# GinZhu/RDST

Hardware: AMD Instinct MI355X
Metric: SR patches/sec fwd+bwd, RDST-E1 x4 64->256 (higher is better)
Workload: dtype bf16; 1 GPU; RDST-E1 x4 (RDST_E1_OASIS_example_SRx4.ini), 1x64x64 LR patches -> 256x256, step = fwd + L1 + bwd + flat-bucket grad all-reduce + Adam; global_batch=32, per_gpu_batch=32, parallelism=dp1, hip_graph=True, grad_bucket_bytes=17859844

## Files before the change

### rdst_amd/csrc/reduce_batch.hip

```cpp
#include "reduce_batch.h"
#include <vector>

namespace rbatch {
namespace {

constexpr int MAXJ = 16;
struct SumBatch { SumJob j[MAXJ]; int first[MAXJ + 1]; int n; };
struct FinBatch { FinJob j[MAXJ]; int first[MAXJ + 1]; int n; };

thread_local bool g_active = false;
thread_local std::vector<SumJob> g_sums;
thread_local std::vector<FinJob> g_fins;

__device__ __forceinline__ void emit(const SumJob& J, int n, int c, int i, float a) {
  if (J.map == MAP_COPY) {
    J.out[J.g4 ? n * J.b2 + c : i] = a;
  } else if (J.map == MAP_LINEAR) {
    const int K = J.a, Kx = J.b;
    if (!J.g4) { n = i / Kx; c = i - n * Kx; }
    if (c < K) { if (J.out) J.out[(int64_t)n * K + c] = a * J.s; }
    else if (c == K && J.out2) J.out2[n] = a * J.s;
  } else if (J.map == MAP_MLP) {
    const int C = J.a, hid = J.b, n1 = hid * (C + 1);
    if (i < n1) J.out[i] = a;
    else {
      const int i2 = i - n1, jj = i2 / C, cc = i2 - jj * C;
      if (jj < hid) J.out2[(int64_t)cc * hid + jj] = a;
      else J.out3[cc] = a;
    }
  } else if (J.map == MAP_T) {
    const int rows = J.a;
    if (n < rows) J.out[(int64_t)c * rows + n] = a;
    else if (n == rows) J.out2[c] = a;
  } else {
    const int heads = J.a, T = J.b, hh = i / T, t = i - hh * T;
    J.out[t * heads + hh] = a;
  }
}

__global__ void __launch_bounds__(256) batched_sum_kernel(const SumBatch bt) {
  __shared__ float part[4][8][33];
  int k = 0;
#pragma unroll
  for (int q = 1; q < MAXJ; ++q) k += (q < bt.n && (int)blockIdx.x >= bt.first[q]) ? 1 : 0;
  const SumJob& J = bt.j[k];
  const int o = threadIdx.x & 31, sg = threadIdx.x >> 5;
  const int i = ((int)blockIdx.x - bt.first[k]) * 32 + o;
  float a0 = 0.f, a1 = 0.f, a2 = 0.f, a3 = 0.f;
  if (i < J.tot) {
    if (J.g4) {
      const uint2* sl = reinterpret_cast<const uint2*>(J.slab);
      for (int w0 = sg; w0 < J.nwg; w0 += 8 * 8) {
        uint2 v[8];
#pragma unroll
        for (int u = 0; u < 8; ++u) v[u] = (w0 + 8 * u < J.nwg) ? sl[(int64_t)(w0 + 8 * u) * J.stride + i] : make_uint2(0u, 0u);
#pragma unroll
        for (int u = 0; u < 8; ++u) {
          a0 += __uint_as_float(v[u].x << 16); a1 += __uint_as_float(v[u].x & 0xffff0000u);
          a2 += __uint_as_float(v[u].y << 16); a3 += __uint_as_float(v[u].y & 0xffff0000u);
        }
      }
    } else {
      for (int w0 = sg; w0 < J.nwg; w0 += 8 * 8) {
        float v[8];
#pragma unroll
        for (int u = 0; u < 8; ++u) v[u] = (w0 + 8 * u < J.nwg) ? J.slab[(int64_t)(w0 + 8 * u) * J.stride + i] : 0.f;
#pragma unroll
        for (int u = 0; u < 8; ++u) a0 += v[u];
      }
    }
  }
  part[0][sg][o] = a0; part[1][sg][o] = a1; part[2][sg][o] = a2; part[3][sg][o] = a3;
  __syncthreads();
  if (sg != 0 || i >= J.tot) return;
  float r[4] = {0.f, 0.f, 0.f, 0.f};
#pragma unroll
  for (int e = 0; e < 4; ++e)
#pragma unroll
    for (int q = 0; q < 8; ++q) r[e] += part[e][q][o];
  if (J.g4) {
    const int W = J.b2, ng = i / W, c = i - ng * W;
#pragma unroll
    for (int e = 0; e < 4; ++e)
      if (4 * ng + e < J.a2) emit(J, 4 * ng + e, c, 0, r[e]);
  } else {
    emit(J, 0, 0, i, r[0]);
  }
}

__global__ void __launch_bounds__(1024) batched_ln_finish_kernel(const FinBatch bt) {
  __shared__ float pg[128][9], pb[128][9], qg[8][9], qb[8][9];
  int kj = 0;
#pragma unroll
  for (int q = 1; q < MAXJ; ++q) kj += (q < bt.n && (int)blockIdx.x >= bt.first[q]) ? 1 : 0;
  const FinJob& J = bt.j[kj];
  const int tx = threadIdx.x & 7, ty = threadIdx.x >> 3;
  const int blk = (int)blockIdx.x - bt.first[kj];
  const int k = blk * 8 + tx;
  const int N = J.N, K = J.K, Kx = J.Kx;
  const float s = J.s;
  const float gk = k < K ? J.gamma[k] : 0.f, bk = k < K ? J.beta[k] : 0.f;
  float ag = 0.f, ab = 0.f;
#pragma unroll 3
  for (int n = ty; n < N; n += 128) {
    const float db = J.G[(int64_t)n * Kx + K];
    if (k < K) {
      const float g = J.G[(int64_t)n * Kx + k], w = J.Wt[(int64_t)n * K + k];
      if (J.dW) J.dW[(int64_t)n * K + k] = s * fmaf(gk, g, bk * db);
      ag = fmaf(w, g, ag);
      ab = fmaf(w, db, ab);
    }
    if (blk == 0 && tx == 0 && J.dbias) J.dbias[n] = s * db;
  }
  pg[ty][tx] = ag;
  pb[ty][tx] = ab;
  __syncthreads();
  if (ty < 8) {
    float a = 0.f, b = 0.f;
#pragma unroll
    for (int j = 0; j < 16; ++j) { a += pg[ty * 16 + j][tx]; b += pb[ty * 16 + j][tx]; }
    qg[ty][tx] = a;
    qb[ty][tx] = b;
  }
  __syncthreads();
  if (ty == 0 && k < K) {
    float a = 0.f, b = 0.f;
#pragma unroll
    for (int j = 0; j < 8; ++j) { a += qg[j][tx]; b += qb[j][tx]; }
    if (J.dgamma) J.dgamma[k] = s * a;
    if (J.dbeta) J.dbeta[k] = s * b;
  }
}

int launch_sums(const SumJob* jobs, int n, hipStream_t st) {
  for (int base = 0; base < n; base += MAXJ) {
    SumBatch bt{};
    bt.n = n - base < MAXJ ? n - base : MAXJ;
    int blocks = 0;
    for (int q = 0; q < bt.n; ++q) {
      bt.j[q] = jobs[base + q];
      bt.first[q] = blocks;
      blocks += (bt.j[q].tot + 31) / 32;
    }
    bt.first[bt.n] = blocks;
    if (blocks == 0) continue;
    hipLaunchKernelGGL(batched_sum_kernel, dim3((unsigned)blocks), dim3(256), 0, st, bt);
    if (int rc = rdst_launch_status("batched_sum")) return rc;
  }
  return 0;
}
int launch_fins(const FinJob* jobs, int n, hipStream_t st) {
  for (int base = 0; base < n; base += MAXJ) {
    FinBatch bt{};
    bt.n = n - base < MAXJ ? n - base : MAXJ;
    int blocks = 0;
    for (int q = 0; q < bt.n; ++q) {
      bt.j[q] = jobs[base + q];
      bt.first[q] = blocks;
      blocks += (bt.j[q].K + 7) / 8;
    }
    bt.first[bt.n] = blocks;
    if (blocks == 0) continue;
    hipLaunchKernelGGL(batched_ln_finish_kernel, dim3((unsigned)blocks), dim3(1024), 0, st, bt);
    if (int rc = rdst_launch_status("batched_ln_finish")) return rc;
  }
  return 0;
}

}

int sum(const SumJob& j, hipStream_t st) {
  if (g_active) { g_sums.push_back(j); return 0; }
  return launch_sums(&j, 1, st);
}
int finish(const FinJob& j, hipStream_t st) {
  if (g_active) { g_fins.push_back(j); return 0; }
  return launch_fins(&j, 1, st);
}

}

extern "C" int rdst_reduce_batch_begin(void) {
  if (rbatch::g_active) return rdst_fail(RDST_EINVAL, "rdst_reduce_batch_begin: a batch is already open on this thread");
  rbatch::g_active = true;
  rbatch::g_sums.clear();
  rbatch::g_fins.clear();
  return 0;
}

extern "C" int rdst_reduce_batch_end(void* stream) {
  if (!rbatch::g_active) return rdst_fail(RDST_EINVAL, "rdst_reduce_batch_end: no open batch");
  rbatch::g_active = false;
  hipStream_t st = (hipStream_t)stream;
  int rc = rbatch::launch_sums(rbatch::g_sums.data(), (int)rbatch::g_sums.size(), st);
  if (!rc) rc = rbatch::launch_fins(rbatch::g_fins.data(), (int)rbatch::g_fins.size(), st);
  rbatch::g_sums.clear();
  rbatch::g_fins.clear();
  return rc;
}

extern "C" int rdst_reduce_batch_abort(void) {
  rbatch::g_active = false;
  rbatch::g_sums.clear();
  rbatch::g_fins.clear();
  return 0;
}
```

Measured before the change: 1889 patches/s.

## Fuse LayerNorm backward finish into batched sum kernel via last-block tickets

Pairs each batched column-sum job with the LayerNorm finish job that consumes its output, and runs both in one kernel launch. Sum blocks are re-tiled per row and column tile; each block bumps a per-chunk atomic ticket in global memory, and the last contributor runs the gamma/beta/dW reduction for that chunk. This removes a separate finish launch and the gap between the two kernels. The cost is atomic traffic, write-through stores with acquire fences, more shared memory per block, and a ticket-slot ring that must stay consistent when the step is replayed from a HIP graph.

```diff
diff --git a/rdst_amd/csrc/reduce_batch.hip b/rdst_amd/csrc/reduce_batch.hip
--- a/rdst_amd/csrc/reduce_batch.hip
+++ b/rdst_amd/csrc/reduce_batch.hip
@@ -1,20 +1,27 @@
 #include "reduce_batch.h"
+#include <atomic>
 #include <vector>
 
 namespace rbatch {
 namespace {
 
 constexpr int MAXJ = 16;
-struct SumBatch { SumJob j[MAXJ]; int first[MAXJ + 1]; int n; };
+constexpr int TICKET_SLOTS = 64;
+struct SumBatch { SumJob j[MAXJ]; FinJob f[MAXJ]; int first[MAXJ + 1]; int n; unsigned paired; int slot; };
 struct FinBatch { FinJob j[MAXJ]; int first[MAXJ + 1]; int n; };
 
 thread_local bool g_active = false;
 thread_local std::vector<SumJob> g_sums;
 thread_local std::vector<FinJob> g_fins;
-
-__device__ __forceinline__ void emit(const SumJob& J, int n, int c, int i, float a) {
+std::atomic<unsigned> g_slot{0};
+constexpr int MAXCH = 32;
+__device__ unsigned g_tickets[TICKET_SLOTS][MAXJ][MAXCH];
+
+__device__ __forceinline__ void emit(const SumJob& J, int n, int c, int i, float a, bool wt) {
   if (J.map == MAP_COPY) {
-    J.out[J.g4 ? n * J.b2 + c : i] = a;
+    float* dst = &J.out[J.g4 ? n * J.b2 + c : i];
+    if (wt) __hip_atomic_store(reinterpret_cast<unsigned*>(dst), __float_as_uint(a), __ATOMIC_RELAXED, __HIP_MEMORY_SCOPE_AGENT);
+    else *dst = a;
   } else if (J.map == MAP_LINEAR) {
     const int K = J.a, Kx = J.b;
     if (!J.g4) { n = i / Kx; c = i - n * Kx; }
@@ -38,16 +45,85 @@
   }
 }
 
-__global__ void __launch_bounds__(256) batched_sum_kernel(const SumBatch bt) {
-  __shared__ float part[4][8][33];
+__device__ __forceinline__ void ln_finish_chunk(const FinJob& J, unsigned q, float* sh) {
+  float* pg = sh; float* pb = sh + 128 * 9; float* qg = sh + 2 * 128 * 9; float* qb = qg + 8 * 9;
+  const unsigned N = J.N, K = J.K, Kx = J.Kx;
+  const float s = J.s;
+  const float* __restrict__ G = J.G;
+  const float* __restrict__ Wt = J.Wt;
+  float* __restrict__ dW = J.dW;
+  float* __restrict__ dbias = J.dbias;
+  const unsigned tx = threadIdx.x & 7, ty0 = threadIdx.x >> 3, k = q * 8 + tx;
+  const unsigned kk = k < K ? k : K - 1;
+  const float gk = J.gamma[kk], bk = J.beta[kk];
+  float ag[4], ab[4];
+#pragma unroll
+  for (int u = 0; u < 4; ++u) ag[u] = ab[u] = 0.f;
+#pragma unroll 1
+  for (unsigned n0 = ty0; n0 < N; n0 += 128) {
+    float gg[4], w[4], db[4];
+#pragma unroll
+    for (int u = 0; u < 4; ++u) {
+      const unsigned n = n0 + 32 * u < N ? n0 + 32 * u : n0;
+      gg[u] = G[n * Kx + kk]; w[u] = Wt[n * K + kk]; db[u] = G[n * Kx + K];
+    }
+#pragma unroll
+    for (int u = 0; u < 4; ++u) {
+      const unsigned n = n0 + 32 * u;
+      if (n < N) {
+        if (k < K) {
+          if (dW) dW[n * K + k] = s * fmaf(gk, gg[u], bk * db[u]);
+          ag[u] = fmaf(w[u], gg[u], ag[u]);
+          ab[u] = fmaf(w[u], db[u], ab[u]);
+        }
+        if (q == 0 && tx == 0 && dbias) dbias[n] = s * db[u];
+      }
+    }
+  }
+#pragma unroll
+  for (int u = 0; u < 4; ++u) { pg[(ty0 + 32 * u) * 9 + tx] = ag[u]; pb[(ty0 + 32 * u) * 9 + tx] = ab[u]; }
+  __syncthreads();
+  if (ty0 < 8) {
+    float a = 0.f, b = 0.f;
+#pragma unroll
+    for (int j = 0; j < 16; ++j) { a += pg[(ty0 * 16 + j) * 9 + tx]; b += pb[(ty0 * 16 + j) * 9 + tx]; }
+    qg[ty0 * 9 + tx] = a;
+    qb[ty0 * 9 + tx] = b;
+  }
+  __syncthreads();
+  if (ty0 == 0 && k < K) {
+    float a = 0.f, b = 0.f;
+#pragma unroll
+    for (int j = 0; j < 8; ++j) { a += qg[j * 9 + tx]; b += qb[j * 9 + tx]; }
+    if (J.dgamma) J.dgamma[k] = s * a;
+    if (J.dbeta) J.dbeta[k] = s * b;
+  }
+  __syncthreads();
+}
+
+constexpr int SH_FIN = 2 * 128 * 9 + 2 * 8 * 9;
+
+__global__ void __launch_bounds__(256, 8) batched_sum_kernel(const SumBatch bt) {
+  __shared__ float sh[SH_FIN + 1];
+  float (*part)[8][33] = reinterpret_cast<float (*)[8][33]>(sh);
   int k = 0;
 #pragma unroll
   for (int q = 1; q < MAXJ; ++q) k += (q < bt.n && (int)blockIdx.x >= bt.first[q]) ? 1 : 0;
   const SumJob& J = bt.j[k];
+  const bool paired = (bt.paired >> k) & 1u;
   const int o = threadIdx.x & 31, sg = threadIdx.x >> 5;
-  const int i = ((int)blockIdx.x - bt.first[k]) * 32 + o;
+  const int blk = (int)blockIdx.x - bt.first[k];
+  int i = blk * 32 + o, tile = 0, units = 0;
+  bool live = i < J.tot;
+  if (paired) {
+    const int W = bt.f[k].Kx, CT = (W + 31) >> 5, r = blk / CT;
+    tile = blk - r * CT;
+    units = (bt.first[k + 1] - bt.first[k]) / CT;
+    live = tile * 32 + o < W;
+    i = r * W + tile * 32 + o;
+  }
   float a0 = 0.f, a1 = 0.f, a2 = 0.f, a3 = 0.f;
-  if (i < J.tot) {
+  if (live) {
     if (J.g4) {
       const uint2* sl = reinterpret_cast<const uint2*>(J.slab);
       for (int w0 = sg; w0 < J.nwg; w0 += 8 * 8) {
@@ -72,19 +148,47 @@
   }
   part[0][sg][o] = a0; part[1][sg][o] = a1; part[2][sg][o] = a2; part[3][sg][o] = a3;
   __syncthreads();
-  if (sg != 0 || i >= J.tot) return;
-  float r[4] = {0.f, 0.f, 0.f, 0.f};
-#pragma unroll
-  for (int e = 0; e < 4; ++e)
-#pragma unroll
-    for (int q = 0; q < 8; ++q) r[e] += part[e][q][o];
-  if (J.g4) {
-    const int W = J.b2, ng = i / W, c = i - ng * W;
+  if (sg == 0 && live) {
+    float r[4] = {0.f, 0.f, 0.f, 0.f};
 #pragma unroll
     for (int e = 0; e < 4; ++e)
-      if (4 * ng + e < J.a2) emit(J, 4 * ng + e, c, 0, r[e]);
-  } else {
-    emit(J, 0, 0, i, r[0]);
+#pragma unroll
+      for (int q = 0; q < 8; ++q) r[e] += part[e][q][o];
+    if (J.g4) {
+      const int W = J.b2, ng = i / W, c = i - ng * W;
+#pragma unroll
+      for (int e = 0; e < 4; ++e)
+        if (4 * ng + e < J.a2) emit(J, 4 * ng + e, c, 0, r[e], paired);
+    } else {
+      emit(J, 0, 0, i, r[0], paired);
+    }
+  }
+  if (!paired) return;
+  if (threadIdx.x < 64) {
+    const FinJob& F = bt.f[k];
+    const int q = threadIdx.x, nch = (F.K + 7) >> 3, tK = F.K >> 5;
+    const bool feeds_q = q < nch && ((q >> 2) == tile || tile == tK);
+    const unsigned want = (unsigned)((q >> 2) == tK ? units : 2 * units);
+    asm volatile("s_waitcnt vmcnt(0)" ::: "memory");
+    bool last = false;
+    if (feeds_q) {
+      unsigned* cnt = &g_tickets[bt.slot][k][q];
+      last = __hip_atomic_fetch_add(cnt, 1u, __ATOMIC_RELAXED, __HIP_MEMORY_SCOPE_AGENT) == want - 1;
+      if (last) __hip_atomic_store(cnt, 0u, __ATOMIC_RELAXED, __HIP_MEMORY_SCOPE_AGENT);
+    }
+    const unsigned mine = (unsigned)__ballot(last);
+    if (mine) {
+      __builtin_amdgcn_fence(__ATOMIC_ACQUIRE, "agent");
+      asm volatile("s_waitcnt vmcnt(0)" ::: "memory");
+    }
+    if (threadIdx.x == 0) sh[SH_FIN] = __uint_as_float(mine);
+  }
+  __syncthreads();
+  unsigned mine = __float_as_uint(sh[SH_FIN]);
+  while (mine) {
+    const unsigned q = __ffs(mine) - 1;
+    mine &= mine - 1;
+    ln_finish_chunk(bt.f[k], q, sh);
   }
 }
 
@@ -132,7 +236,7 @@
   }
 }
 
-int launch_sums(const SumJob* jobs, int n, hipStream_t st) {
+int launch_sums(const SumJob* jobs, const FinJob* fins, int n, hipStream_t st) {
   for (int base = 0; base < n; base += MAXJ) {
     SumBatch bt{};
     bt.n = n - base < MAXJ ? n - base : MAXJ;
@@ -140,10 +244,17 @@
     for (int q = 0; q < bt.n; ++q) {
       bt.j[q] = jobs[base + q];
       bt.first[q] = blocks;
-      blocks += (bt.j[q].tot + 31) / 32;
+      if (fins && fins[base + q].G) {
+        bt.f[q] = fins[base + q];
+        bt.paired |= 1u << q;
+        blocks += (bt.j[q].g4 ? (bt.j[q].a2 + 3) / 4 : bt.f[q].N) * ((bt.f[q].Kx + 31) / 32);
+      } else {
+        blocks += (bt.j[q].tot + 31) / 32;
+      }
     }
     bt.first[bt.n] = blocks;
     if (blocks == 0) continue;
+    if (bt.paired) bt.slot = (int)(g_slot.fetch_add(1u, std::memory_order_relaxed) % TICKET_SLOTS);
     hipLaunchKernelGGL(batched_sum_kernel, dim3((unsigned)blocks), dim3(256), 0, st, bt);
     if (int rc = rdst_launch_status("batched_sum")) return rc;
   }
@@ -167,11 +278,39 @@
   return 0;
 }
 
+bool feeds(const SumJob& sj, const FinJob& fj) {
+  if (sj.map != MAP_COPY || sj.out != fj.G || fj.Kx != fj.K + 1 || fj.N <= 0 || fj.K <= 0 || fj.K > 8 * MAXCH) return false;
+  return sj.g4 ? (sj.a2 == fj.N && sj.b2 == fj.Kx) : (sj.tot == fj.N * fj.Kx);
+}
+
+int launch_paired(hipStream_t st) {
+  const int ns = (int)g_sums.size();
+  std::vector<int> fin_of(ns, -1);
+  std::vector<FinJob> rest;
+  for (size_t f = 0; f < g_fins.size(); ++f) {
+    int hit = -1;
+    for (int q = ns - 1; q >= 0 && hit < 0; --q)
+      if (fin_of[q] < 0 && feeds(g_sums[q], g_fins[f])) hit = q;
+    if (hit >= 0) fin_of[hit] = (int)f; else rest.push_back(g_fins[f]);
+  }
+  std::vector<SumJob> sums;
+  std::vector<FinJob> fins;
+  for (int pass = 0; pass < 2; ++pass)
+    for (int q = 0; q < ns; ++q)
+      if ((fin_of[q] >= 0) == (pass == 0)) {
+        sums.push_back(g_sums[q]);
+        fins.push_back(fin_of[q] >= 0 ? g_fins[fin_of[q]] : FinJob{});
+      }
+  int rc = launch_sums(sums.data(), fins.data(), ns, st);
+  if (!rc) rc = launch_fins(rest.data(), (int)rest.size(), st);
+  return rc;
+}
+
 }
 
 int sum(const SumJob& j, hipStream_t st) {
   if (g_active) { g_sums.push_back(j); return 0; }
-  return launch_sums(&j, 1, st);
+  return launch_sums(&j, nullptr, 1, st);
 }
 int finish(const FinJob& j, hipStream_t st) {
   if (g_active) { g_fins.push_back(j); return 0; }
@@ -192,8 +331,7 @@
   if (!rbatch::g_active) return rdst_fail(RDST_EINVAL, "rdst_reduce_batch_end: no open batch");
   rbatch::g_active = false;
   hipStream_t st = (hipStream_t)stream;
-  int rc = rbatch::launch_sums(rbatch::g_sums.data(), (int)rbatch::g_sums.size(), st);
-  if (!rc) rc = rbatch::launch_fins(rbatch::g_fins.data(), (int)rbatch::g_fins.size(), st);
+  int rc = rbatch::launch_paired(st);
   rbatch::g_sums.clear();
   rbatch::g_fins.clear();
   return rc;
```

Result: slower. 1834 patches/s (-2.9%).
